# wg-perception/tod

Measured on AMD Instinct MI355X. Metric: frames/sec @ 640x480, 1M-descriptor DB; achieved HBM GB/s on BF-matcher, higher is better.
Workload: dtype fp4 (+-1) x fp4 -> f32 on the matrix cores (exact integers), f32 in the verifier

## Files before the change

include/todhip.h:

```cpp
#ifndef TODHIP_H_
#define TODHIP_H_

#include <stddef.h>
#include <stdint.h>

#ifdef __cplusplus
extern "C" {
#endif

#define TODHIP_VERSION 1

typedef enum {
  TODHIP_OK = 0,
  TODHIP_EINVAL = -1,
  TODHIP_ENODB = -2,
  TODHIP_EHIP = -3,
  TODHIP_ECAPACITY = -4,
  TODHIP_ERANGE = -5,
  TODHIP_ENOMEM = -6,
  TODHIP_ESCRATCH = -7,
  TODHIP_EBUSY = -8,
  TODHIP_ETIMEOUT = -9
} todhip_status;

// ... 3 lines not shown

typedef struct { int32_t queryIdx, trainIdx, imgIdx; float distance; } todhip_dmatch;

typedef struct { uint32_t s[31]; uint32_t f, b; uint64_t draws; } todhip_rng;

typedef struct { uint32_t min_inliers, n_ransac_iterations; float sensor_error; } todhip_verify_params;

typedef struct { uint32_t object; float R[9]; float t[3]; uint32_t inlier_begin, inlier_end; } todhip_pose;

typedef struct {
  uint64_t db_rows, db_objects;
  uint32_t last_nq, last_k, last_matches;
  uint32_t last_objects_verified, last_rounds, last_hypotheses, last_gate_calls, last_poses;
  double   last_match_kernel_ms;
  double   sum_match_kernel_ms;
  uint64_t n_match_kernel_launches;
  uint32_t last_sprint_launches;
  uint32_t last_sprint_rounds;
  uint32_t last_verify_ticks;
  uint32_t last_block_split;
  uint64_t k4x_half_blocks, k4x_half_blocks_completed;
  uint32_t last_fp4_rows;
  uint32_t fp4_rows_builds;
} todhip_counters;

int  todhip_version(void);
int  todhip_create(int device, void* hip_stream, todhip_ctx** out);
void todhip_destroy(todhip_ctx*);
void* todhip_stream(todhip_ctx*);
int  todhip_last_hip_error(const todhip_ctx*);
int  todhip_synchronize(todhip_ctx*);
int  todhip_get_counters(todhip_ctx*, todhip_counters* out);
enum { TODHIP_STREAM_THROUGHPUT = 0, TODHIP_STREAM_LATENCY = 1 };
int  todhip_set_cu_partition(uint32_t latency_cus);
int  todhip_stream_create(int device, int kind, void** stream_out);
int  todhip_stream_destroy(void* stream);
int  todhip_set_kernel_timing(todhip_ctx*, int enable);
enum { TODHIP_ENGINE_AUTO = 0, TODHIP_ENGINE_VALU = 1, TODHIP_ENGINE_MFMA = 2 };
int  todhip_set_matcher_engine(todhip_ctx*, int engine);
int  todhip_set_matcher_block_split(todhip_ctx*, int split);

int todhip_db_load(todhip_ctx*, const todhip_object* objs, uint32_t n_objs, uint32_t desc_bytes,
                   uint32_t shard_rank, uint32_t shard_count, float* spans_out);
int todhip_db_load_device(todhip_ctx*, const todhip_object* objs, uint32_t n_objs, uint32_t desc_bytes,
                          uint32_t shard_rank, uint32_t shard_count, float* spans_out);
int todhip_db_info(const todhip_ctx*, uint64_t* total_rows, uint64_t* shard_first_row, uint64_t* shard_rows,
// ... 251 lines not shown
```

tod_amd/capi.py:

```python
import ctypes as C
import os
import subprocess

import numpy as np

_PKG = os.path.dirname(os.path.abspath(__file__))
LIB_PATH = os.environ.get("TODHIP_LIB_PATH") or os.path.join(_PKG, "libtodhip.so")

OK, EINVAL, ENODB, EHIP, ECAPACITY, ERANGE, ENOMEM, ESCRATCH, EBUSY, ETIMEOUT = 0, -1, -2, -3, -4, -5, -6, -7, -8, -9
FRAME_GRAY8, FRAME_BGR8, FRAME_BGRA8 = 0, 1, 2
PATTERN_ORDER_RANK, PATTERN_ORDER_MATCHER = 0, 1

DMATCH_DTYPE = np.dtype([("queryIdx", "<i4"), ("trainIdx", "<i4"), ("imgIdx", "<i4"), ("distance", "<f4")])


class TodObject(C.Structure):
    _fields_ = [("desc", C.c_void_p), ("pts_xyz", C.c_void_p), ("n", C.c_uint32)]


class Rng(C.Structure):
    _fields_ = [("s", C.c_uint32 * 31), ("f", C.c_uint32), ("b", C.c_uint32), ("draws", C.c_uint64)]


class VerifyParams(C.Structure):
    _fields_ = [("min_inliers", C.c_uint32), ("n_ransac_iterations", C.c_uint32), ("sensor_error", C.c_float)]


class Pose(C.Structure):
    _fields_ = [("object", C.c_uint32), ("R", C.c_float * 9), ("t", C.c_float * 3),
                ("inlier_begin", C.c_uint32), ("inlier_end", C.c_uint32)]


class RoundTrace(C.Structure):
    _fields_ = [("object", C.c_uint32), ("iterations", C.c_uint32), ("best_iteration", C.c_uint32),
                ("best_count", C.c_int32), ("draws_before", C.c_uint64), ("draws_after", C.c_uint64),
                ("n_inlier_kp", C.c_uint32), ("accepted", C.c_uint32)]


class Counters(C.Structure):
    _fields_ = [("db_rows", C.c_uint64), ("db_objects", C.c_uint64), ("last_nq", C.c_uint32), ("last_k", C.c_uint32),
                ("last_matches", C.c_uint32), ("last_objects_verified", C.c_uint32), ("last_rounds", C.c_uint32),
                ("last_hypotheses", C.c_uint32), ("last_gate_calls", C.c_uint32), ("last_poses", C.c_uint32),
                ("last_match_kernel_ms", C.c_double), ("sum_match_kernel_ms", C.c_double),
                ("n_match_kernel_launches", C.c_uint64), ("last_sprint_launches", C.c_uint32), ("last_sprint_rounds", C.c_uint32),
                ("last_verify_ticks", C.c_uint32), ("last_block_split", C.c_uint32), ("k4x_half_blocks", C.c_uint64),
                ("k4x_half_blocks_completed", C.c_uint64), ("last_fp4_rows", C.c_uint32), ("fp4_rows_builds", C.c_uint32)]


class PipelineParams(C.Structure):
    _fields_ = [("struct_size", C.c_uint32), ("frames_per_step", C.c_uint32), ("H", C.c_uint32), ("W", C.c_uint32),
                ("frame_format", C.c_int), ("depth_is_u16", C.c_int), ("K9", C.c_float * 9), ("n_features", C.c_uint32),
                ("n_levels", C.c_uint32), ("scale_factor", C.c_float), ("k", C.c_uint32), ("radius", C.c_uint32),
                ("verify", VerifyParams), ("rng_seed", C.c_uint32), ("orb_workers", C.c_uint32), ("verify_workers", C.c_uint32),
                ("ring_depth", C.c_uint32), ("max_poses_per_frame", C.c_uint32)]


class PipelineStats(C.Structure):
    _fields_ = [("steps", C.c_uint64), ("frames", C.c_uint64), ("keypoints", C.c_uint64), ("poses", C.c_uint64),
                ("orb_s", C.c_double), ("match_issue_s", C.c_double), ("verify_s", C.c_double),
                ("sum_match_kernel_ms", C.c_double), ("n_match_kernel_launches", C.c_uint64)]


class PatternStats(C.Structure):
    _fields_ = [("n_keypoints", C.c_uint32), ("n_candidates", C.c_uint32), ("accepted_in_round", C.c_uint32 * 6)]


EXPORTS = [
    "todhip_version", "todhip_create", "todhip_destroy", "todhip_stream", "todhip_last_hip_error",
    "todhip_synchronize", "todhip_get_counters", "todhip_set_cu_partition", "todhip_stream_create", "todhip_stream_destroy", "todhip_set_kernel_timing", "todhip_set_matcher_engine", "todhip_set_matcher_block_split", "todhip_set_ratio_test", "todhip_db_load", "todhip_db_load_device", "todhip_db_info",
# ... 961 lines not shown
```

tod_amd/csrc/capi.hip:

```cpp
#include <algorithm>
#include <atomic>
#include <cfloat>
#include <cmath>
#include <cstring>
#include <cstdlib>
#include <new>
#include <vector>

#include "ctx.h"

extern "C" {

int todhip_version(void) { return TODHIP_VERSION; }

int todhip_create(int device, void* hip_stream, todhip_ctx** out) {
  if (!out) return TODHIP_EINVAL;
  *out = nullptr;
  todhip_ctx* ctx = new (std::nothrow) todhip_ctx();
  if (!ctx) return TODHIP_ENOMEM;
  ctx->device = device;
  hipError_t e = hipSetDevice(device);
  if (e == hipSuccess) {
    hipDeviceProp_t prop;
    if (hipGetDeviceProperties(&prop, device) == hipSuccess && prop.multiProcessorCount > 0)
// ... 287 lines not shown
  return tod_match_shard_keys(ctx, d_q_desc, nq, k, radius, reinterpret_cast<uint64_t*>(d_keys));
}

int todhip_merge_shards_device_on(todhip_ctx* ctx, void* hip_stream, const void* d_keys_all, uint32_t n_shards, uint32_t nq,
                                  uint32_t k, uint32_t radius, void* d_counts, void* d_matches, void* d_matches_xyz) {
  if (!ctx || !hip_stream) return TODHIP_EINVAL;
  return merge_shards(ctx, reinterpret_cast<hipStream_t>(hip_stream), d_keys_all, n_shards, nq, k, radius, d_counts, d_matches, d_matches_xyz);
}

int todhip_merge_shards_device(todhip_ctx* ctx, const void* d_keys_all, uint32_t n_shards, uint32_t nq, uint32_t k,
                               uint32_t radius, void* d_counts, void* d_matches, void* d_matches_xyz) {
  return merge_shards(ctx, nullptr, d_keys_all, n_shards, nq, k, radius, d_counts, d_matches, d_matches_xyz);
}

int todhip_match_device(todhip_ctx* ctx, const void* d_q_desc, uint32_t nq, uint32_t k, uint32_t radius,
                        void* d_counts, void* d_matches, void* d_matches_xyz) {
  if (!ctx || !d_q_desc || !d_counts || !d_matches || !d_matches_xyz) return TODHIP_EINVAL;
  if (k == 0 || k > 8 || radius == 0) return TODHIP_EINVAL;
  if (ctx->total_rows == 0) return TODHIP_ENODB;
  if (ctx->shard_rows != ctx->total_rows) return TODHIP_EINVAL;
  if (wide_db_with_lsh(ctx)) return TODHIP_EINVAL;
  if (nq == 0) return TODHIP_OK;
  const uint32_t k_in = (ctx->ratio > 0.f && k < 2) ? 2u : k;
  TOD_HIP(ctx->m_keys.reserve(tod_match_lists_bytes(nq, k_in)));
  uint32_t n_lists = 0;
  int rc = tod_match_lists(ctx, d_q_desc, nq, k_in, radius, ctx->m_keys.as<uint64_t>(), &n_lists);
  if (rc != TODHIP_OK) return rc;
  rc = tod_match_finalize(ctx, ctx->m_keys.as<uint64_t>(), n_lists, nq, k_in, k, radius,
                          reinterpret_cast<uint32_t*>(d_counts), reinterpret_cast<todhip_dmatch*>(d_matches),
                          reinterpret_cast<float*>(d_matches_xyz));
  if (rc == TODHIP_OK && ctx->cross_check_q)
    rc = tod_cross_check(ctx, d_q_desc, nq, ctx->cross_check_q, nullptr, k, reinterpret_cast<uint32_t*>(d_counts),
                         reinterpret_cast<todhip_dmatch*>(d_matches), reinterpret_cast<float*>(d_matches_xyz));
  if (rc == TODHIP_OK) { ctx->counters.last_nq = nq; ctx->counters.last_k = k; }
  return rc;
}

int todhip_match(todhip_ctx* ctx, const uint8_t* q_desc, uint32_t nq, uint32_t k, uint32_t radius,
                 uint32_t* row_ptr, todhip_dmatch* matches, float* matches_xyz) {
  if (!ctx || !row_ptr || (nq && (!q_desc || !matches || !matches_xyz))) return TODHIP_EINVAL;
  if (k == 0 || k > 8 || radius == 0) return TODHIP_EINVAL;
  if (ctx->total_rows == 0) return TODHIP_ENODB;
  if (wide_db_with_lsh(ctx)) return TODHIP_EINVAL;
  if (nq == 0) { row_ptr[0] = 0; return TODHIP_OK; }
  TOD_HIP(hipSetDevice(ctx->device));
  const size_t nm = (size_t)nq * k;
  TOD_HIP(ctx->m_q.reserve((size_t)nq * ctx->desc_bytes));
  TOD_HIP(ctx->m_counts.reserve((size_t)nq * sizeof(uint32_t)));
  TOD_HIP(ctx->m_matches.reserve(nm * sizeof(todhip_dmatch)));
  TOD_HIP(ctx->m_xyz.reserve(nm * 3 * sizeof(float)));
  const size_t stage_bytes = (size_t)nq * sizeof(uint32_t) + nm * sizeof(todhip_dmatch) + nm * 3 * sizeof(float);
  TOD_HIP(ctx->h_stage.reserve(stage_bytes));
  TOD_HIP(hipMemcpyAsync(ctx->m_q.p, q_desc, (size_t)nq * ctx->desc_bytes, hipMemcpyHostToDevice, ctx->stream));
// ... 35 lines not shown
```

tod_amd/csrc/ctx.h:

```cpp
#pragma once

#include <hip/hip_runtime.h>

#include <cstdint>
#include <cstdlib>
#include <cstring>
#include <memory>
#include <type_traits>
#include <vector>

#include "../../include/todhip.h"
#include "db_select.h"
#include "fp4_rows.h"
#include "match_split.h"
#include "match_tiles.h"

#define TOD_HIP(call)                                  \
  do {                                                 \
    hipError_t e_ = (call);                            \
    if (e_ != hipSuccess) {                            \
      ctx->last_hip_error = (int)e_;                   \
      return TODHIP_EHIP;                              \
    }                                                  \
  } while (0)

#ifndef TOD_LATENCY_PRIO_LEVEL
#define TOD_LATENCY_PRIO_LEVEL 3
#endif
#define TOD_LATENCY_PRIO() __builtin_amdgcn_s_setprio(TOD_LATENCY_PRIO_LEVEL)

constexpr size_t kDbSlackBytes = 2048;
static_assert(31 * 64 <= kDbSlackBytes, "a 32-row step of the widest binary row must end inside the slack");

struct DevBuf {
  void* p = nullptr;
  size_t cap = 0;
// ... 48 lines not shown
  template <typename T> T* as() const { return reinterpret_cast<T*>(p); }
};

struct TodWs { virtual ~TodWs() {} };
enum TodWsSlot { kWsVerify, kWsOrb, kWsL2, kWsPnp, kWsLsh, kWsLearn, kWsCompact, kWsRadius, kWsCrossCheck, kWsSlots };

struct todhip_ctx {
  int device = 0;
  hipStream_t stream = nullptr;
  bool own_stream = false;
  int last_hip_error = 0;
  int n_cu = 256;

  uint32_t desc_bytes = 0;
  uint64_t total_rows = 0, shard_first = 0, shard_rows = 0;
  uint32_t n_objs = 0;
  DevBuf db_desc;
  DevBuf db_pts;
  DevBuf db_obj_off;
  std::vector<uint32_t> h_obj_off;
  std::vector<float> h_spans;

  DevBuf m_q, m_part, m_keys, m_counts, m_matches, m_xyz, m_bound;
  HostBuf h_stage;
  bool time_kernels = false;
  static constexpr int kEvPairs = 64;
  hipEvent_t evp[2 * kEvPairs] = {};
  uint64_t ev_head = 0, ev_tail = 0;
  todhip_counters counters = {};
  int matcher_engine = TODHIP_ENGINE_AUTO;
  HostBuf k4x_stats_host; DevBuf k4x_stats_dev;
  K4xSplit k4x;
  float ratio = 0.f;
  uint32_t cross_check_q = 0;
  int bit_order_mode = TODHIP_BIT_ORDER_NONE;
  bool bit_order_on = false;
  uint8_t bit_src_of[256];
  DevBuf bit_tab, m_qord;
  bool sel_on = false;
  TodViewTables sel;
  DevBuf view_desc, view_tab;
  DevBuf db_fp4;
  uint64_t rows_gen = 1, fp4_gen = 0;

  std::vector<todhip_round_trace> traces;

// ... 18 lines not shown
  r.s[r.f] += r.s[r.b];
  const uint32_t out = r.s[r.f] >> 1;
  r.f = r.f == 30u ? 0u : r.f + 1u; r.b = r.b == 30u ? 0u : r.b + 1u;
  ++r.draws;
  return out;
}

uint32_t tod_pack_csr(const uint32_t* counts, const todhip_dmatch* m, const float* xyz, uint32_t nq, uint32_t k, uint32_t* row_ptr,
                      todhip_dmatch* matches, float* matches_xyz);
extern "C" hipError_t tod_stream_create(hipStream_t* out, int device, int kind);
extern "C" uint32_t tod_cu_partition();
int tod_timing_begin(todhip_ctx* ctx, int* slot);
int tod_timing_end(todhip_ctx* ctx, int slot);
int tod_timing_drain(todhip_ctx* ctx, uint64_t keep);
struct KernelTimer {
  todhip_ctx* ctx;
  int slot = -1;
  int begin() { return ctx->time_kernels ? tod_timing_begin(ctx, &slot) : TODHIP_OK; }
  int end() { return slot >= 0 ? tod_timing_end(ctx, slot) : TODHIP_OK; }
};
int tod_match_lists(todhip_ctx* ctx, const void* d_q, uint32_t nq, uint32_t k, uint32_t radius, uint64_t* d_lists,
                    uint32_t* n_lists);
size_t tod_match_lists_bytes(uint32_t nq, uint32_t k);
int tod_wide_lists_active(todhip_ctx* ctx, const void* d_q, uint32_t nq, uint32_t k, uint32_t radius, uint64_t* d_lists,
                          uint32_t* n_lists);
template <typename Fn>
int dispatch_k(uint32_t k, Fn fn) {
  switch (k) {
    case 1: return fn(std::integral_constant<int, 1>{});
    case 2: return fn(std::integral_constant<int, 2>{});
    case 3: return fn(std::integral_constant<int, 3>{});
    case 4: return fn(std::integral_constant<int, 4>{});
    case 5: return fn(std::integral_constant<int, 5>{});
    case 6: return fn(std::integral_constant<int, 6>{});
    case 7: return fn(std::integral_constant<int, 7>{});
    case 8: return fn(std::integral_constant<int, 8>{});
    default: return TODHIP_EINVAL;
  }
}
int tod_match_shard_keys(todhip_ctx* ctx, const void* d_q, uint32_t nq, uint32_t k, uint32_t radius, uint64_t* d_keys);
int tod_match_finalize(todhip_ctx* ctx, const uint64_t* d_keys_all, uint32_t n_shards, uint32_t nq, uint32_t k_in, uint32_t k_out,
                       uint32_t radius, uint32_t* d_counts, todhip_dmatch* d_matches, float* d_xyz,
                       hipStream_t stream = nullptr);
int tod_cross_check(todhip_ctx* ctx, const void* d_q, uint32_t nq, uint32_t frame_queries, const uint32_t* frame_nq, uint32_t stride,
                    uint32_t* d_counts, todhip_dmatch* d_matches, float* d_xyz);
int tod_cluster_frames_nocloud(todhip_ctx* ctx, uint32_t F, const float* d_kp_xy, uint32_t nq, const uint32_t* d_counts,
// ... 17 lines not shown
```

tod_amd/csrc/match.hip:

```cpp
#include <algorithm>
#include <cstdio>
#include <cstdlib>
#include <cstring>

#include "ctx.h"
#include "row_ops.h"

namespace {

#include "match_keys.h"
#include "match_valu.h"
#include "match_fp4.h"
#include "match_mfma.h"
#include "match_pair_pack.h"
#include "match_fp4rows.h"
#include "match_merge.h"
#include "match_plan.h"
#include "match_launch.h"

int k4_engine(const todhip_ctx* ctx, uint32_t nq) {
  if (ctx->matcher_engine == TODHIP_ENGINE_VALU) return 0;
  if (ctx->matcher_engine == TODHIP_ENGINE_MFMA) return 1;
  if (match_env().engine == 'v') return 0;
  if (match_env().engine == 'm') return 1;
  return (uint64_t)nq * tod_db_n_rows(ctx) >= (1ull << 24) ? 1 : 0;
}

}

int tod_timing_drain(todhip_ctx* ctx, uint64_t keep) {
  while (ctx->ev_head - ctx->ev_tail > keep) {
    const int i = (int)(ctx->ev_tail % todhip_ctx::kEvPairs);
    TOD_HIP(hipEventSynchronize(ctx->evp[2 * i + 1]));
    float ms = 0.f;
    TOD_HIP(hipEventElapsedTime(&ms, ctx->evp[2 * i], ctx->evp[2 * i + 1]));
    ctx->counters.last_match_kernel_ms = ms;
    ctx->counters.sum_match_kernel_ms += ms;
    ctx->counters.n_match_kernel_launches += 1;
    ++ctx->ev_tail;
  }
// ... 19 lines not shown
  const uint32_t* q = reinterpret_cast<const uint32_t*>(d_q);
  return dispatch_k(k, [&](auto K) { return launch_topk<decltype(K)::value>(ctx, q, nq, radius, d_lists, n_lists); });
}

int tod_match_lists(todhip_ctx* ctx, const void* d_q, uint32_t nq, uint32_t k, uint32_t radius, uint64_t* d_lists,
                    uint32_t* n_lists) {
  const bool wide = ctx->desc_bytes == 64;
  if ((!wide && ctx->desc_bytes != 32) || k == 0 || k > 8 || nq == 0) return TODHIP_EINVAL;
  if (wide && tod_lsh_enabled(ctx)) return TODHIP_EINVAL;
  if (!wide && ctx->bit_order_on) {
    int rc = tod_bit_order_queries(ctx, d_q, nq, &d_q);
    if (rc != TODHIP_OK) return rc;
  }
  if (tod_db_n_rows(ctx) == 0) {
    TOD_HIP(hipMemsetAsync(d_lists, 0xFF, (size_t)nq * k * sizeof(uint64_t), ctx->stream));
    *n_lists = 1;
    return TODHIP_OK;
  }
  int rc = wide ? tod_wide_lists_active(ctx, d_q, nq, k, radius, d_lists, n_lists) : match_lists_active(ctx, d_q, nq, k, radius, d_lists, n_lists);
  if (rc != TODHIP_OK || !ctx->sel_on) return rc;
  return tod_view_remap(ctx, d_lists, (size_t)*n_lists * nq * k);
}

size_t tod_match_lists_bytes(uint32_t nq, uint32_t k) { return (size_t)kMergeGroups * nq * k * sizeof(uint64_t); }

int tod_match_shard_keys(todhip_ctx* ctx, const void* d_q, uint32_t nq, uint32_t k, uint32_t radius, uint64_t* d_keys) {
  if (nq == 0) return TODHIP_OK;
  if (tod_db_n_rows(ctx) == 0) {
    TOD_HIP(hipMemsetAsync(d_keys, 0xFF, (size_t)nq * k * sizeof(uint64_t), ctx->stream));
    return TODHIP_OK;
  }
  TOD_HIP(ctx->m_keys.reserve(tod_match_lists_bytes(nq, k)));
  uint32_t n_lists = 0;
  int rc = tod_match_lists(ctx, d_q, nq, k, radius, ctx->m_keys.as<uint64_t>(), &n_lists);
  if (rc != TODHIP_OK) return rc;
  hipLaunchKernelGGL(select_keys_kernel, dim3((nq + kBlock - 1) / kBlock), dim3(kBlock), 0, ctx->stream,
                     ctx->m_keys.as<uint64_t>(), n_lists, nq, k, d_keys);
  TOD_HIP(hipGetLastError());
  return TODHIP_OK;
}

int tod_match_finalize(todhip_ctx* ctx, const uint64_t* d_keys_all, uint32_t n_shards, uint32_t nq, uint32_t k_in, uint32_t k_out,
                       uint32_t radius, uint32_t* d_counts, todhip_dmatch* d_matches, float* d_xyz, hipStream_t stream) {
  if (nq == 0) return TODHIP_OK;
  const uint32_t blocks = (nq + kBlock - 1) / kBlock;
  hipLaunchKernelGGL(finalize_kernel, dim3(blocks), dim3(kBlock), 0, stream ? stream : ctx->stream, d_keys_all, n_shards, nq, k_in, k_out,
// ... 16 lines not shown
```

tod_amd/csrc/match_launch.h:

```cpp

int k4_engine(const todhip_ctx* ctx, uint32_t nq);

struct MatchEnv {
  char engine;
  int k4_mode;
  int k4_wpc;
  int k4x_wpc;
  int k4x_share;
  int k4x_qt;
  int k4x_half;
  bool k4x_half_debug;
  int k4x_fp4_rows;
  int k4x_fp4_rows_mb;
  int k4x_pairs;
};
inline const MatchEnv& match_env() {
  static const MatchEnv env = [] {
    auto num = [](const char* name, int unset) { const char* e = getenv(name); return e ? atoi(e) : unset; };
    const char* eng = getenv("TODHIP_K4_ENGINE");
    return MatchEnv{eng ? eng[0] : '\0', num("TODHIP_K4_MODE", -1), num("TODHIP_K4_WAVES_PER_CU", 0), num("TODHIP_K4X_WAVES_PER_CU", 0),
                    num("TODHIP_K4X_SHARE", 16), num("TODHIP_K4X_QT", 0), num("TODHIP_K4X_HALF", -1), getenv("TODHIP_K4X_HALF_DEBUG") != nullptr,
                    num("TODHIP_K4X_FP4_ROWS", 1), num("TODHIP_K4X_FP4_ROWS_MB", 512), num("TODHIP_K4X_PAIRS", 1)};
  }();
  return env;
}

inline int fp4_rows_ready(todhip_ctx* ctx, uint32_t n_rows, const uint4** out) {
  const MatchEnv& env = match_env();
  const size_t bytes = fp4_rows_bytes(n_rows);
  if (env.k4x_fp4_rows == 0 || bytes > ((size_t)std::max(0, env.k4x_fp4_rows_mb) << 20) || bytes >= (1ull << 32)) return TODHIP_OK;
  if (ctx->fp4_gen != ctx->rows_gen) {
    TOD_HIP(ctx->db_fp4.reserve(bytes));
    hipLaunchKernelGGL(expand_rows_fp4_kernel, dim3(fp4_rows_steps(n_rows)), dim3(kBlock), 0, ctx->stream,
                       reinterpret_cast<const uint32_t*>(tod_db_rows(ctx)), fp4_rows_steps(n_rows), ctx->db_fp4.as<uint4>());
    TOD_HIP(hipGetLastError());
    ctx->fp4_gen = ctx->rows_gen;
    ++ctx->counters.fp4_rows_builds;
  }
  *out = ctx->db_fp4.as<uint4>();
  return TODHIP_OK;
}

template <int K, int QT>
int launch_topk_mfma_qt(todhip_ctx* ctx, const uint32_t* d_q, uint32_t nq, uint32_t radius, uint64_t* d_lists, uint32_t* n_lists) {
  constexpr bool PF2 = QT < 8;
  const MatchEnv& env = match_env();
  const uint32_t cut = radius >= 256u ? kNoLimit : radius + 1u;
  const uint32_t n_rows = (uint32_t)tod_db_n_rows(ctx);
  const uint32_t n_qw = (nq + 32u * QT - 1u) / (32u * QT), n_qw64 = (nq + 63u) / 64u;
  const uint32_t nq_pad = n_qw64 * 64u;
  uint32_t wpc = 32;
  if ((uint64_t)n_rows * n_qw < (uint64_t)ctx->n_cu * wpc * 1536u) wpc = 16;
  if ((uint64_t)n_rows * n_qw < (uint64_t)ctx->n_cu * 16u * 4096u) wpc = 8;
  if (env.k4x_wpc > 0) wpc = (uint32_t)env.k4x_wpc;
  Tiling t;
  if (!finish_tiling(n_rows, mfma_tile_rows(n_rows, (uint32_t)ctx->n_cu * wpc / n_qw, 256u, true), n_qw, &t)) return TODHIP_EINVAL;
  uint8_t* const d_stored = prepare_lists<K>(ctx, t.n_tiles, nq_pad, n_qw64);
  if (!d_stored) return TODHIP_EHIP;
  KernelTimer timer{ctx};
  if (int rc = timer.begin()) return rc;
  const uint32_t min_split = QT < 4 ? 4u : (cut <= 64u ? 2u : (cut <= 96u ? 3u : 4u));
  if (ctx->k4x.may_split(min_split, env.k4x_half)) {
    if (!ctx->k4x_stats_host.p) {
      TOD_HIP(ctx->k4x_stats_host.reserve(64));
      std::memset(ctx->k4x_stats_host.p, 0, 64);
      TOD_HIP(ctx->k4x_stats_dev.reserve(64));
      TOD_HIP(hipMemsetAsync(ctx->k4x_stats_dev.p, 0, 64, ctx->stream));
    }
    ctx->k4x.take_report(ctx->k4x_stats_host.as<uint32_t>(), ctx->counters, min_split, env.k4x_half, env.k4x_half_debug);
  }
  const uint32_t split = ctx->k4x.next(min_split, env.k4x_half);
  const bool pairs = env.k4x_pairs != 0 && (QT == 6 || nq <= 1024u);
  const int mode = split == 2 ? (pairs ? 2 : 4) : split == 3 ? 3 : cut <= 128u ? 1 : 0;
  ctx->counters.last_block_split = split;
  uint32_t* const d_stats = split < 4 ? ctx->k4x_stats_dev.as<uint32_t>() : nullptr;
  const uint4* rows_fp4 = nullptr;
  if ((QT == 4 || QT == 6) && t.rows_per_tile % 32u == 0u)
    if (int rc = fp4_rows_ready(ctx, n_rows, &rows_fp4)) return rc;
  ctx->counters.last_fp4_rows = rows_fp4 ? 1u : 0u;
  auto launch = [&](auto kern, auto rows) {
    hipLaunchKernelGGL(kern, dim3(t.blocks_per_xcd * 8u), dim3(kBlock), 0, ctx->stream, rows, d_q, n_rows, nq, nq_pad, t.rows_per_tile,
                       t.n_tiles, n_qw, n_qw64, t.blocks_per_xcd, t.tiles_per_xcd, cut, (uint32_t)std::max(2, env.k4x_share),
                       ctx->m_part.as<uint32_t>(), ctx->m_bound.as<uint32_t>(), d_stored, d_stats ? d_stats + 2u * (split - 2u) : nullptr);
  };
  auto launch_mode = [&](auto M) {
    constexpr int MODE = decltype(M)::value;
    if constexpr (QT == 4 || QT == 6)
      if (rows_fp4) return launch(hamming_topk_fp4rows<K, QT, MODE>, rows_fp4);
    launch(hamming_topk_mfma<K, QT, MODE == 4 ? 2 : MODE, PF2>, reinterpret_cast<const uint32_t*>(tod_db_rows(ctx)));
  };
  switch (mode) {
    case 0: launch_mode(std::integral_constant<int, 0>{}); break;
    case 1: launch_mode(std::integral_constant<int, 1>{}); break;
    case 2: launch_mode(std::integral_constant<int, 2>{}); break;
    case 4: launch_mode(std::integral_constant<int, 4>{}); break;
    default: launch_mode(std::integral_constant<int, 3>{}); break;
  }
  if (int rc = timer.end()) return rc;
  if (d_stats) ++ctx->k4x.seq_sent;
  if (nq <= 64u && !d_stats && t.n_tiles >= 256u) return launch_merge_wave<K>(ctx, nq, nq_pad, t, d_stored, n_qw64, d_lists, n_lists);
  return launch_merge<K>(ctx, nq, nq_pad, t, d_stored, n_qw64, d_stats, d_lists, n_lists);
}

template <int K>
int launch_topk_mfma_q32(todhip_ctx* ctx, const uint32_t* d_q, uint32_t nq, uint32_t radius, uint64_t* d_lists, uint32_t* n_lists) {
  const uint32_t cut = radius >= 256u ? kNoLimit : radius + 1u;
  const uint32_t n_rows = (uint32_t)tod_db_n_rows(ctx), n_qw64 = 1u, nq_pad = 64u;
  Tiling t;
  if (!finish_tiling(n_rows, mfma_tile_rows(n_rows, (uint32_t)ctx->n_cu * 32u, 2048u, false), 1u, &t)) return TODHIP_EINVAL;
  uint8_t* const d_stored = prepare_lists<K>(ctx, t.n_tiles, nq_pad, n_qw64);
  if (!d_stored) return TODHIP_EHIP;
  KernelTimer timer{ctx};
  if (int rc = timer.begin()) return rc;
  auto kern = cut <= 128u ? hamming_topk_mfma_q32<K, true> : hamming_topk_mfma_q32<K, false>;
  ctx->counters.last_fp4_rows = 0;
  hipLaunchKernelGGL(kern, dim3((t.n_tiles + kWavesPerBlock - 1) / kWavesPerBlock), dim3(kBlock), 0, ctx->stream,
                     reinterpret_cast<const uint32_t*>(tod_db_rows(ctx)), d_q, n_rows, nq, nq_pad, t.rows_per_tile, t.n_tiles, n_qw64, cut,
                     (uint32_t)std::max(4, match_env().k4x_share), ctx->m_part.as<uint32_t>(), ctx->m_bound.as<uint32_t>(), d_stored);
  if (int rc = timer.end()) return rc;
  return launch_merge_wave<K>(ctx, nq, nq_pad, t, d_stored, n_qw64, d_lists, n_lists);
}

template <int K>
int launch_topk_mfma(todhip_ctx* ctx, const uint32_t* d_q, uint32_t nq, uint32_t radius, uint64_t* d_lists, uint32_t* n_lists) {
  const int env_qt = match_env().k4x_qt;
  if (nq <= 32u && !(env_qt > 0))
    return launch_topk_mfma_q32<K>(ctx, d_q, nq, radius, d_lists, n_lists);
  constexpr int kMaxQT = K <= 2 ? 8 : (K <= 5 ? 6 : 4);
  auto padded = [&](uint32_t qt) { return (uint64_t)((nq + 32u * qt - 1u) / (32u * qt) * (32u * qt)); };
  int qt = kMaxQT >= 6 ? 6 : 4;
  if (kMaxQT >= 8 && padded(8) * 103u < padded(6) * 100u) qt = 8;
  if (qt > 4 && padded(4) * 103u < padded((uint32_t)qt) * 100u) qt = 4;
  if (padded(2) * 103u < padded((uint32_t)qt) * 100u) qt = 2;
  if (nq <= 2048u && qt > 4) qt = 4;
  if ((env_qt == 2 || env_qt == 4 || env_qt == 6 || env_qt == 8) && env_qt <= kMaxQT) qt = env_qt;
  if (qt == 8) return launch_topk_mfma_qt<K, (kMaxQT >= 8 ? 8 : 4)>(ctx, d_q, nq, radius, d_lists, n_lists);
  if (qt == 6) return launch_topk_mfma_qt<K, (kMaxQT >= 6 ? 6 : 4)>(ctx, d_q, nq, radius, d_lists, n_lists);
  if (qt == 2) return launch_topk_mfma_qt<K, 2>(ctx, d_q, nq, radius, d_lists, n_lists);
  return launch_topk_mfma_qt<K, 4>(ctx, d_q, nq, radius, d_lists, n_lists);
}

template <int K>
int launch_topk(todhip_ctx* ctx, const uint32_t* d_q, uint32_t nq, uint32_t radius, uint64_t* d_lists, uint32_t* n_lists) {
  if (k4_engine(ctx, nq) == 1) return launch_topk_mfma<K>(ctx, d_q, nq, radius, d_lists, n_lists);
  const MatchEnv& env = match_env();
  const uint32_t cut = radius >= 256u ? 0xFFFFFFFFu : radius + 1u;
  const uint32_t n_rows = (uint32_t)tod_db_n_rows(ctx);
  const uint32_t n_qw = (nq + 63u) / 64u;
  const uint32_t nq_pad = n_qw * 64u;
  uint32_t n_tiles;
  if (env.k4_wpc > 0) {
    n_tiles = (uint32_t)ctx->n_cu * (uint32_t)env.k4_wpc / n_qw;
  } else {
    n_tiles = std::max(3u * (uint32_t)ctx->n_cu * (uint32_t)kWavesPerCU / n_qw, (n_rows + 2047u) / 2048u);
    n_tiles = std::min(n_tiles, 8192u);
  }
  if (n_tiles < 1) n_tiles = 1;
  if (n_tiles >= 8) n_tiles = (n_tiles + 7u) & ~7u;
  uint32_t rows_per_tile = (n_rows + n_tiles - 1) / n_tiles;
  rows_per_tile = ((rows_per_tile + 2 * kGroupRows - 1) / (2 * kGroupRows)) * (2 * kGroupRows);
  if (rows_per_tile < 64) rows_per_tile = 64;
  Tiling t;
// ... 16 lines not shown
```

tod_amd/csrc/match_merge.h:

```cpp

template <int K>
__global__ __launch_bounds__(kBlock) void merge_tiles_kernel(const uint32_t* __restrict__ part, uint32_t nq,
                                                             uint32_t nq_pad, uint32_t n_tiles,
                                                             uint32_t rows_per_tile, uint64_t first_global_row,
                                                             uint32_t n_groups, const uint8_t* __restrict__ stored,
                                                             uint32_t n_qw, uint64_t* __restrict__ keys,
                                                             const uint32_t* stat_src = nullptr, uint32_t* stat_dst = nullptr,
                                                             uint32_t stat_seq = 0) {
  TOD_LATENCY_PRIO();
  const uint32_t qi = blockIdx.x * kBlock + threadIdx.x;
  const uint32_t grp = blockIdx.y;
  if (stat_dst && qi == 0u && grp == 0u) {
    for (int i = 0; i < 4; ++i) stat_dst[i] = __hip_atomic_load(stat_src + i, __ATOMIC_RELAXED, __HIP_MEMORY_SCOPE_AGENT);
    __threadfence_system();
    stat_dst[4] = stat_seq;
  }
  if (qi >= nq) return;
  uint64_t best[K];
#pragma unroll
  for (int j = 0; j < K; ++j) best[j] = ~0ull;
#pragma unroll 4
  for (uint32_t t = grp; t < n_tiles; t += n_groups) {
    if (stored[(size_t)t * n_qw + (qi >> 6)] != 0) continue;
    uint32_t pk[K];
// ... 57 lines not shown
    for (int j = 0; j < K; ++j) keys[((size_t)grp * nq + qi) * K + j] = best[j];
  }
}

__global__ __launch_bounds__(kBlock) void select_keys_kernel(const uint64_t* __restrict__ lists, uint32_t n_lists,
                                                             uint32_t nq, uint32_t k, uint64_t* __restrict__ keys) {
  TOD_LATENCY_PRIO();
  const uint32_t qi = blockIdx.x * kBlock + threadIdx.x;
  if (qi >= nq) return;
  uint64_t last = 0;
  bool have_last = false;
  for (uint32_t j = 0; j < k; ++j) {
    const uint64_t nxt = next_key_over_lists(lists, n_lists, nq, qi, k, last, have_last);
    keys[(size_t)qi * k + j] = nxt;
    if (nxt == ~0ull) {
      for (uint32_t jj = j + 1; jj < k; ++jj) keys[(size_t)qi * k + jj] = ~0ull;
      break;
    }
    last = nxt;
    have_last = true;
  }
}

__global__ __launch_bounds__(kBlock) void finalize_kernel(const uint64_t* __restrict__ keys_all, uint32_t n_shards,
                                                          uint32_t nq, uint32_t k_in, uint32_t k_out, uint32_t radius, float ratio,
                                                          const uint32_t* __restrict__ obj_off, uint32_t n_objs,
                                                          const float* __restrict__ pts,
                                                          uint32_t* __restrict__ counts,
                                                          todhip_dmatch* __restrict__ matches,
                                                          float* __restrict__ xyz) {
  TOD_LATENCY_PRIO();
  const uint32_t qi = blockIdx.x * kBlock + threadIdx.x;
  if (qi >= nq) return;
  uint64_t picked[9];
  const uint32_t want = ratio > 0.f ? max(k_out, 2u) : k_out;
  uint32_t n_picked = 0;
  uint64_t last = 0;
  bool have_last = false;
  for (uint32_t j = 0; j < want; ++j) {
    const uint64_t nxt = next_key_over_lists(keys_all, n_shards, nq, qi, k_in, last, have_last);
    if (nxt == ~0ull) break;
    last = nxt;
    have_last = true;
    picked[n_picked++] = nxt;
  }
  if (ratio > 0.f && n_picked >= 2u && !((float)(uint32_t)(picked[0] >> 32) < ratio * (float)(uint32_t)(picked[1] >> 32))) n_picked = 0;
  uint32_t kept = 0;
  for (uint32_t j = 0; j < n_picked && j < k_out; ++j) {
    const uint32_t d = (uint32_t)(picked[j] >> 32);
    if ((float)d > (float)radius) break;
    store_match(qi, d, (uint32_t)picked[j], (size_t)qi * k_out + kept, obj_off, n_objs, pts, matches, xyz);
    ++kept;
  }
  counts[qi] = kept;
}
```

tod_amd/csrc/match_plan.h:

```cpp

inline bool finish_tiling(uint32_t n_rows, uint32_t rows_per_tile, uint32_t n_qw, Tiling* t) {
  if (rows_per_tile > kLocalMask) return false;
  *t = tile_plan(n_rows, rows_per_tile, n_qw, kWavesPerBlock, kMergeGroups);
  return true;
}

template <int K>
uint8_t* prepare_lists(todhip_ctx* ctx, uint32_t n_tiles, uint32_t nq_pad, uint32_t n_qw64) {
  const size_t bound_bytes = (size_t)nq_pad * sizeof(uint32_t), flag_bytes = (size_t)n_tiles * n_qw64;
  hipError_t e = ctx->m_part.reserve((size_t)n_tiles * K * nq_pad * sizeof(uint32_t));
  if (e == hipSuccess) e = ctx->m_bound.reserve(bound_bytes + flag_bytes);
  if (e == hipSuccess) e = hipMemsetAsync(ctx->m_bound.p, 0xFF, bound_bytes + flag_bytes, ctx->stream);
  if (e != hipSuccess) { ctx->last_hip_error = (int)e; return nullptr; }
  return ctx->m_bound.as<uint8_t>() + bound_bytes;
}

template <int K>
int launch_merge(todhip_ctx* ctx, uint32_t nq, uint32_t nq_pad, const Tiling& t, const uint8_t* d_stored, uint32_t n_qw64,
                 const uint32_t* d_stats, uint64_t* d_lists, uint32_t* n_lists) {
  hipLaunchKernelGGL(merge_tiles_kernel<K>, dim3((nq + kBlock - 1) / kBlock, t.groups), dim3(kBlock), 0, ctx->stream,
                     ctx->m_part.as<uint32_t>(), nq, nq_pad, t.n_tiles, t.rows_per_tile, tod_db_first_row(ctx), t.groups, d_stored, n_qw64, d_lists,
                     d_stats, d_stats ? ctx->k4x_stats_host.as<uint32_t>() : (uint32_t*)nullptr, d_stats ? ctx->k4x.seq_sent : 0u);
  TOD_HIP(hipGetLastError());
  *n_lists = t.groups;
  return TODHIP_OK;
}

template <int K>
int launch_merge_wave(todhip_ctx* ctx, uint32_t nq, uint32_t nq_pad, const Tiling& t, const uint8_t* d_stored, uint32_t n_qw64,
                      uint64_t* d_lists, uint32_t* n_lists) {
  hipLaunchKernelGGL(merge_tiles_wave_kernel<K>, dim3((nq + kWavesPerBlock - 1) / kWavesPerBlock, t.groups), dim3(kBlock), 0, ctx->stream,
                     ctx->m_part.as<uint32_t>(), nq, nq_pad, t.n_tiles, t.rows_per_tile, tod_db_first_row(ctx), t.groups, d_stored, n_qw64, d_lists);
  TOD_HIP(hipGetLastError());
  *n_lists = t.groups;
  return TODHIP_OK;
}
// ... 1 lines not shown
```

Before: 25040.

## Fuse tile merge with finalize epilogue and skip per-call bound memset

Adds a direct MFMA match path that merges per-tile top-K partials and writes final DMatch/xyz output in one kernel, instead of writing intermediate 64-bit lists and running a separate finalize kernel. The fused kernel also restores the bound/stored-flag buffer to 0xFF on exit, so the next call can skip the hipMemsetAsync when the buffer is already clean. This removes one kernel launch, a global round trip of the list buffer, and a memset per frame. The cost is extra coupling: correctness now depends on the previous fused kernel having fully reset the scratch flags.

```diff
diff --git a/include/todhip.h b/include/todhip.h
--- a/include/todhip.h
+++ b/include/todhip.h
@@ -49,6 +49,8 @@
   uint64_t k4x_half_blocks, k4x_half_blocks_completed;
   uint32_t last_fp4_rows;
   uint32_t fp4_rows_builds;
+  uint32_t last_match_epilogue;
+  uint32_t bound_memsets;
 } todhip_counters;
 
 int  todhip_version(void);
diff --git a/tod_amd/capi.py b/tod_amd/capi.py
--- a/tod_amd/capi.py
+++ b/tod_amd/capi.py
@@ -44,7 +44,8 @@
                 ("last_match_kernel_ms", C.c_double), ("sum_match_kernel_ms", C.c_double),
                 ("n_match_kernel_launches", C.c_uint64), ("last_sprint_launches", C.c_uint32), ("last_sprint_rounds", C.c_uint32),
                 ("last_verify_ticks", C.c_uint32), ("last_block_split", C.c_uint32), ("k4x_half_blocks", C.c_uint64),
-                ("k4x_half_blocks_completed", C.c_uint64), ("last_fp4_rows", C.c_uint32), ("fp4_rows_builds", C.c_uint32)]
+                ("k4x_half_blocks_completed", C.c_uint64), ("last_fp4_rows", C.c_uint32), ("fp4_rows_builds", C.c_uint32),
+                ("last_match_epilogue", C.c_uint32), ("bound_memsets", C.c_uint32)]
 
 
 class PipelineParams(C.Structure):
diff --git a/tod_amd/csrc/capi.hip b/tod_amd/csrc/capi.hip
--- a/tod_amd/csrc/capi.hip
+++ b/tod_amd/csrc/capi.hip
@@ -333,13 +333,19 @@
   if (wide_db_with_lsh(ctx)) return TODHIP_EINVAL;
   if (nq == 0) return TODHIP_OK;
   const uint32_t k_in = (ctx->ratio > 0.f && k < 2) ? 2u : k;
-  TOD_HIP(ctx->m_keys.reserve(tod_match_lists_bytes(nq, k_in)));
-  uint32_t n_lists = 0;
-  int rc = tod_match_lists(ctx, d_q_desc, nq, k_in, radius, ctx->m_keys.as<uint64_t>(), &n_lists);
+  bool done = false;
+  int rc = tod_match_direct(ctx, d_q_desc, nq, k_in, k, radius, reinterpret_cast<uint32_t*>(d_counts),
+                            reinterpret_cast<todhip_dmatch*>(d_matches), reinterpret_cast<float*>(d_matches_xyz), &done);
   if (rc != TODHIP_OK) return rc;
-  rc = tod_match_finalize(ctx, ctx->m_keys.as<uint64_t>(), n_lists, nq, k_in, k, radius,
-                          reinterpret_cast<uint32_t*>(d_counts), reinterpret_cast<todhip_dmatch*>(d_matches),
-                          reinterpret_cast<float*>(d_matches_xyz));
+  if (!done) {
+    TOD_HIP(ctx->m_keys.reserve(tod_match_lists_bytes(nq, k_in)));
+    uint32_t n_lists = 0;
+    rc = tod_match_lists(ctx, d_q_desc, nq, k_in, radius, ctx->m_keys.as<uint64_t>(), &n_lists);
+    if (rc != TODHIP_OK) return rc;
+    rc = tod_match_finalize(ctx, ctx->m_keys.as<uint64_t>(), n_lists, nq, k_in, k, radius,
+                            reinterpret_cast<uint32_t*>(d_counts), reinterpret_cast<todhip_dmatch*>(d_matches),
+                            reinterpret_cast<float*>(d_matches_xyz));
+  }
   if (rc == TODHIP_OK && ctx->cross_check_q)
     rc = tod_cross_check(ctx, d_q_desc, nq, ctx->cross_check_q, nullptr, k, reinterpret_cast<uint32_t*>(d_counts),
                          reinterpret_cast<todhip_dmatch*>(d_matches), reinterpret_cast<float*>(d_matches_xyz));
diff --git a/tod_amd/csrc/ctx.h b/tod_amd/csrc/ctx.h
--- a/tod_amd/csrc/ctx.h
+++ b/tod_amd/csrc/ctx.h
@@ -12,6 +12,7 @@
 #include "../../include/todhip.h"
 #include "db_select.h"
 #include "fp4_rows.h"
+#include "match_bound_extent.h"
 #include "match_split.h"
 #include "match_tiles.h"
 
@@ -106,6 +107,7 @@
   std::vector<float> h_spans;
 
   DevBuf m_q, m_part, m_keys, m_counts, m_matches, m_xyz, m_bound;
+  BoundExtent m_bound_clean;
   HostBuf h_stage;
   bool time_kernels = false;
   static constexpr int kEvPairs = 64;
@@ -170,6 +172,8 @@
 int tod_match_lists(todhip_ctx* ctx, const void* d_q, uint32_t nq, uint32_t k, uint32_t radius, uint64_t* d_lists,
                     uint32_t* n_lists);
 size_t tod_match_lists_bytes(uint32_t nq, uint32_t k);
+int tod_match_direct(todhip_ctx* ctx, const void* d_q, uint32_t nq, uint32_t k_in, uint32_t k_out, uint32_t radius, uint32_t* d_counts,
+                     todhip_dmatch* d_matches, float* d_xyz, bool* done);
 int tod_wide_lists_active(todhip_ctx* ctx, const void* d_q, uint32_t nq, uint32_t k, uint32_t radius, uint64_t* d_lists,
                           uint32_t* n_lists);
 template <typename Fn>
diff --git a/tod_amd/csrc/match.hip b/tod_amd/csrc/match.hip
--- a/tod_amd/csrc/match.hip
+++ b/tod_amd/csrc/match.hip
@@ -16,6 +16,7 @@
 #include "match_fp4rows.h"
 #include "match_merge.h"
 #include "match_plan.h"
+#include "match_epilogue.h"
 #include "match_launch.h"
 
 int k4_engine(const todhip_ctx* ctx, uint32_t nq) {
@@ -81,6 +82,30 @@
   return tod_view_remap(ctx, d_lists, (size_t)*n_lists * nq * k);
 }
 
+int tod_match_direct(todhip_ctx* ctx, const void* d_q, uint32_t nq, uint32_t k_in, uint32_t k_out, uint32_t radius, uint32_t* d_counts,
+                     todhip_dmatch* d_matches, float* d_xyz, bool* done) {
+  *done = false;
+  ctx->counters.last_match_epilogue = 0;
+  if (match_env().epilogue == 0 || ctx->desc_bytes != 32 || k_in == 0 || k_in > 8 || nq == 0) return TODHIP_OK;
+  if (tod_lsh_enabled(ctx) || ctx->sel_on || tod_db_n_rows(ctx) == 0) return TODHIP_OK;
+  if (k4_engine(ctx, nq) != 1 || !mfma_takes_qt(nq)) return TODHIP_OK;
+  if (ctx->bit_order_on) {
+    int rc = tod_bit_order_queries(ctx, d_q, nq, &d_q);
+    if (rc != TODHIP_OK) return rc;
+  }
+  MatchOut out{k_out, radius, d_counts, d_matches, d_xyz, false};
+  const uint32_t search_radius = ctx->ratio > 0.f ? 256u : radius;
+  const uint32_t* q = reinterpret_cast<const uint32_t*>(d_q);
+  uint32_t n_lists = 0;
+  int rc = dispatch_k(k_in, [&](auto K) { return launch_topk_mfma<decltype(K)::value>(ctx, q, nq, search_radius, nullptr, &n_lists, &out); });
+  if (rc != TODHIP_OK) return rc;
+  if (!out.taken)
+    rc = tod_match_finalize(ctx, ctx->m_keys.as<uint64_t>(), n_lists, nq, k_in, k_out, radius, d_counts, d_matches, d_xyz);
+  ctx->counters.last_match_epilogue = out.taken ? 1u : 0u;
+  *done = true;
+  return rc;
+}
+
 size_t tod_match_lists_bytes(uint32_t nq, uint32_t k) { return (size_t)kMergeGroups * nq * k * sizeof(uint64_t); }
 
 int tod_match_shard_keys(todhip_ctx* ctx, const void* d_q, uint32_t nq, uint32_t k, uint32_t radius, uint64_t* d_keys) {
diff --git a/tod_amd/csrc/match_bound_extent.h b/tod_amd/csrc/match_bound_extent.h
--- /dev/null
+++ b/tod_amd/csrc/match_bound_extent.h
@@ -0,0 +1,19 @@
+#pragma once
+#include <algorithm>
+#include <cstddef>
+
+struct BoundExtent {
+  size_t clean = 0;
+  size_t held = 0;
+
+  void reallocated() { clean = held = 0; }
+
+  bool begin(size_t need, bool restoring) {
+    const bool fill = !restoring || need > clean;
+    held = restoring ? std::max(clean, need) : 0;
+    clean = 0;
+    return fill;
+  }
+
+  void restored() { clean = held; held = 0; }
+};
diff --git a/tod_amd/csrc/match_epilogue.h b/tod_amd/csrc/match_epilogue.h
--- /dev/null
+++ b/tod_amd/csrc/match_epilogue.h
@@ -0,0 +1,93 @@
+
+constexpr int kEpiGroups = 4;
+
+struct MatchOut {
+  uint32_t k_out, radius;
+  uint32_t* counts;
+  todhip_dmatch* matches;
+  float* xyz;
+  bool taken;
+};
+
+template <int K>
+__global__ __launch_bounds__(kBlock) void merge_finalize_kernel(const uint32_t* __restrict__ part, uint32_t nq, uint32_t nq_pad, uint32_t n_tiles,
+                                                                uint32_t rows_per_tile, uint64_t first_global_row, uint8_t* stored,
+                                                                uint32_t n_qw64, uint32_t* bound, uint32_t k_out, uint32_t radius, float ratio,
+                                                                const uint32_t* __restrict__ obj_off, uint32_t n_objs,
+                                                                const float* __restrict__ pts, uint32_t* __restrict__ counts,
+                                                                todhip_dmatch* __restrict__ matches, float* __restrict__ xyz,
+                                                                const uint32_t* stat_src, uint32_t* stat_dst, uint32_t stat_seq) {
+  TOD_LATENCY_PRIO();
+  static_assert(kBlock == 64 * kEpiGroups, "a workgroup is 64 queries x kEpiGroups tile groups");
+  __shared__ uint64_t lists[kEpiGroups * K * 64];
+  const uint32_t q = threadIdx.x & 63u, grp = threadIdx.x >> 6, qw = blockIdx.x;
+  const uint32_t qi = qw * 64u + q;
+  if (stat_dst && threadIdx.x == 0u && qw == 0u) {
+    for (int i = 0; i < 4; ++i) stat_dst[i] = __hip_atomic_load(stat_src + i, __ATOMIC_RELAXED, __HIP_MEMORY_SCOPE_AGENT);
+    __threadfence_system();
+    stat_dst[4] = stat_seq;
+  }
+  uint64_t best[K];
+#pragma unroll
+  for (int j = 0; j < K; ++j) best[j] = ~0ull;
+  if (qi < nq) {
+#pragma unroll 4
+    for (uint32_t t = grp; t < n_tiles; t += kEpiGroups) {
+      if (stored[(size_t)t * n_qw64 + qw] != 0) continue;
+      uint32_t pk[K];
+#pragma unroll
+      for (int j = 0; j < K; ++j) pk[j] = part[((size_t)t * K + j) * nq_pad + qi];
+#pragma unroll
+      for (int j = 0; j < K; ++j) {
+        uint64_t key = pk[j] == 0xFFFFFFFFu
+                           ? ~0ull
+                           : (((uint64_t)(pk[j] >> kLocalBits) << 32) |
+                              (first_global_row + (uint64_t)t * rows_per_tile + (pk[j] & kLocalMask)));
+#pragma unroll
+        for (int s2 = 0; s2 < K; ++s2) {
+          uint64_t lo = key < best[s2] ? key : best[s2];
+          key = key < best[s2] ? best[s2] : key;
+          best[s2] = lo;
+        }
+      }
+    }
+  }
+#pragma unroll
+  for (int j = 0; j < K; ++j) lists[(grp * K + j) * 64u + q] = best[j];
+  __syncthreads();
+  if (grp == 0u && qi < nq) {
+    uint64_t picked[9];
+    const uint32_t want = ratio > 0.f ? max(k_out, 2u) : k_out;
+    uint32_t n_picked = 0, heads = 0;
+    for (uint32_t j = 0; j < want; ++j) {
+      uint64_t nxt = ~0ull;
+      uint32_t from = 0;
+#pragma unroll
+      for (uint32_t g = 0; g < (uint32_t)kEpiGroups; ++g) {
+        const uint32_t h = (heads >> (8u * g)) & 0xFFu;
+        if (h >= (uint32_t)K) continue;
+        const uint64_t v = lists[(g * K + h) * 64u + q];
+        if (v < nxt) { nxt = v; from = g; }
+      }
+      if (nxt == ~0ull) break;
+      heads += 1u << (8u * from);
+      picked[n_picked++] = nxt;
+    }
+    finalize_tail(qi, picked, n_picked, k_out, radius, ratio, obj_off, n_objs, pts, counts, matches, xyz);
+  }
+  for (uint32_t t = threadIdx.x; t < n_tiles; t += kBlock) stored[(size_t)t * n_qw64 + qw] = 0xFFu;
+  if (threadIdx.x < 64u) bound[qi] = 0xFFFFFFFFu;
+}
+
+template <int K>
+int launch_merge_finalize(todhip_ctx* ctx, uint32_t nq, uint32_t nq_pad, const Tiling& t, uint8_t* d_stored, uint32_t n_qw64,
+                          const uint32_t* d_stats, MatchOut* out) {
+  hipLaunchKernelGGL(merge_finalize_kernel<K>, dim3(n_qw64), dim3(kBlock), 0, ctx->stream, ctx->m_part.as<uint32_t>(), nq, nq_pad, t.n_tiles,
+                     t.rows_per_tile, tod_db_first_row(ctx), d_stored, n_qw64, ctx->m_bound.as<uint32_t>(), out->k_out, out->radius, ctx->ratio,
+                     ctx->db_obj_off.as<uint32_t>(), ctx->n_objs, ctx->db_pts.as<float>(), out->counts, out->matches, out->xyz, d_stats,
+                     d_stats ? ctx->k4x_stats_host.as<uint32_t>() : (uint32_t*)nullptr, d_stats ? ctx->k4x.seq_sent : 0u);
+  TOD_HIP(hipGetLastError());
+  ctx->m_bound_clean.restored();
+  out->taken = true;
+  return TODHIP_OK;
+}
diff --git a/tod_amd/csrc/match_launch.h b/tod_amd/csrc/match_launch.h
--- a/tod_amd/csrc/match_launch.h
+++ b/tod_amd/csrc/match_launch.h
@@ -13,6 +13,7 @@
   int k4x_fp4_rows;
   int k4x_fp4_rows_mb;
   int k4x_pairs;
+  int epilogue;
 };
 inline const MatchEnv& match_env() {
   static const MatchEnv env = [] {
@@ -20,7 +21,7 @@
     const char* eng = getenv("TODHIP_K4_ENGINE");
     return MatchEnv{eng ? eng[0] : '\0', num("TODHIP_K4_MODE", -1), num("TODHIP_K4_WAVES_PER_CU", 0), num("TODHIP_K4X_WAVES_PER_CU", 0),
                     num("TODHIP_K4X_SHARE", 16), num("TODHIP_K4X_QT", 0), num("TODHIP_K4X_HALF", -1), getenv("TODHIP_K4X_HALF_DEBUG") != nullptr,
-                    num("TODHIP_K4X_FP4_ROWS", 1), num("TODHIP_K4X_FP4_ROWS_MB", 512), num("TODHIP_K4X_PAIRS", 1)};
+                    num("TODHIP_K4X_FP4_ROWS", 1), num("TODHIP_K4X_FP4_ROWS_MB", 512), num("TODHIP_K4X_PAIRS", 1), num("TODHIP_MATCH_EPILOGUE", 1)};
   }();
   return env;
 }
@@ -42,7 +43,8 @@
 }
 
 template <int K, int QT>
-int launch_topk_mfma_qt(todhip_ctx* ctx, const uint32_t* d_q, uint32_t nq, uint32_t radius, uint64_t* d_lists, uint32_t* n_lists) {
+int launch_topk_mfma_qt(todhip_ctx* ctx, const uint32_t* d_q, uint32_t nq, uint32_t radius, uint64_t* d_lists, uint32_t* n_lists,
+                        MatchOut* direct = nullptr) {
   constexpr bool PF2 = QT < 8;
   const MatchEnv& env = match_env();
   const uint32_t cut = radius >= 256u ? kNoLimit : radius + 1u;
@@ -55,10 +57,6 @@
   if (env.k4x_wpc > 0) wpc = (uint32_t)env.k4x_wpc;
   Tiling t;
   if (!finish_tiling(n_rows, mfma_tile_rows(n_rows, (uint32_t)ctx->n_cu * wpc / n_qw, 256u, true), n_qw, &t)) return TODHIP_EINVAL;
-  uint8_t* const d_stored = prepare_lists<K>(ctx, t.n_tiles, nq_pad, n_qw64);
-  if (!d_stored) return TODHIP_EHIP;
-  KernelTimer timer{ctx};
-  if (int rc = timer.begin()) return rc;
   const uint32_t min_split = QT < 4 ? 4u : (cut <= 64u ? 2u : (cut <= 96u ? 3u : 4u));
   if (ctx->k4x.may_split(min_split, env.k4x_half)) {
     if (!ctx->k4x_stats_host.p) {
@@ -70,10 +68,16 @@
     ctx->k4x.take_report(ctx->k4x_stats_host.as<uint32_t>(), ctx->counters, min_split, env.k4x_half, env.k4x_half_debug);
   }
   const uint32_t split = ctx->k4x.next(min_split, env.k4x_half);
+  uint32_t* const d_stats = split < 4 ? ctx->k4x_stats_dev.as<uint32_t>() : nullptr;
+  const bool wave_merge = nq <= 64u && !d_stats && t.n_tiles >= 256u;
+  const bool fused = direct && !wave_merge;
+  uint8_t* const d_stored = prepare_lists<K>(ctx, t.n_tiles, nq_pad, n_qw64, fused);
+  if (!d_stored) return TODHIP_EHIP;
+  KernelTimer timer{ctx};
+  if (int rc = timer.begin()) return rc;
   const bool pairs = env.k4x_pairs != 0 && (QT == 6 || nq <= 1024u);
   const int mode = split == 2 ? (pairs ? 2 : 4) : split == 3 ? 3 : cut <= 128u ? 1 : 0;
   ctx->counters.last_block_split = split;
-  uint32_t* const d_stats = split < 4 ? ctx->k4x_stats_dev.as<uint32_t>() : nullptr;
   const uint4* rows_fp4 = nullptr;
   if ((QT == 4 || QT == 6) && t.rows_per_tile % 32u == 0u)
     if (int rc = fp4_rows_ready(ctx, n_rows, &rows_fp4)) return rc;
@@ -98,7 +102,12 @@
   }
   if (int rc = timer.end()) return rc;
   if (d_stats) ++ctx->k4x.seq_sent;
-  if (nq <= 64u && !d_stats && t.n_tiles >= 256u) return launch_merge_wave<K>(ctx, nq, nq_pad, t, d_stored, n_qw64, d_lists, n_lists);
+  if (fused) return launch_merge_finalize<K>(ctx, nq, nq_pad, t, d_stored, n_qw64, d_stats, direct);
+  if (direct) {
+    TOD_HIP(ctx->m_keys.reserve(tod_match_lists_bytes(nq, K)));
+    d_lists = ctx->m_keys.as<uint64_t>();
+  }
+  if (wave_merge) return launch_merge_wave<K>(ctx, nq, nq_pad, t, d_stored, n_qw64, d_lists, n_lists);
   return launch_merge<K>(ctx, nq, nq_pad, t, d_stored, n_qw64, d_stats, d_lists, n_lists);
 }
 
@@ -121,10 +130,13 @@
   return launch_merge_wave<K>(ctx, nq, nq_pad, t, d_stored, n_qw64, d_lists, n_lists);
 }
 
+inline bool mfma_takes_qt(uint32_t nq) { return nq > 32u || match_env().k4x_qt > 0; }
+
 template <int K>
-int launch_topk_mfma(todhip_ctx* ctx, const uint32_t* d_q, uint32_t nq, uint32_t radius, uint64_t* d_lists, uint32_t* n_lists) {
+int launch_topk_mfma(todhip_ctx* ctx, const uint32_t* d_q, uint32_t nq, uint32_t radius, uint64_t* d_lists, uint32_t* n_lists,
+                     MatchOut* direct = nullptr) {
   const int env_qt = match_env().k4x_qt;
-  if (nq <= 32u && !(env_qt > 0))
+  if (!mfma_takes_qt(nq))
     return launch_topk_mfma_q32<K>(ctx, d_q, nq, radius, d_lists, n_lists);
   constexpr int kMaxQT = K <= 2 ? 8 : (K <= 5 ? 6 : 4);
   auto padded = [&](uint32_t qt) { return (uint64_t)((nq + 32u * qt - 1u) / (32u * qt) * (32u * qt)); };
@@ -134,10 +146,10 @@
   if (padded(2) * 103u < padded((uint32_t)qt) * 100u) qt = 2;
   if (nq <= 2048u && qt > 4) qt = 4;
   if ((env_qt == 2 || env_qt == 4 || env_qt == 6 || env_qt == 8) && env_qt <= kMaxQT) qt = env_qt;
-  if (qt == 8) return launch_topk_mfma_qt<K, (kMaxQT >= 8 ? 8 : 4)>(ctx, d_q, nq, radius, d_lists, n_lists);
-  if (qt == 6) return launch_topk_mfma_qt<K, (kMaxQT >= 6 ? 6 : 4)>(ctx, d_q, nq, radius, d_lists, n_lists);
-  if (qt == 2) return launch_topk_mfma_qt<K, 2>(ctx, d_q, nq, radius, d_lists, n_lists);
-  return launch_topk_mfma_qt<K, 4>(ctx, d_q, nq, radius, d_lists, n_lists);
+  if (qt == 8) return launch_topk_mfma_qt<K, (kMaxQT >= 8 ? 8 : 4)>(ctx, d_q, nq, radius, d_lists, n_lists, direct);
+  if (qt == 6) return launch_topk_mfma_qt<K, (kMaxQT >= 6 ? 6 : 4)>(ctx, d_q, nq, radius, d_lists, n_lists, direct);
+  if (qt == 2) return launch_topk_mfma_qt<K, 2>(ctx, d_q, nq, radius, d_lists, n_lists, direct);
+  return launch_topk_mfma_qt<K, 4>(ctx, d_q, nq, radius, d_lists, n_lists, direct);
 }
 
 template <int K>
diff --git a/tod_amd/csrc/match_merge.h b/tod_amd/csrc/match_merge.h
--- a/tod_amd/csrc/match_merge.h
+++ b/tod_amd/csrc/match_merge.h
@@ -103,6 +103,21 @@
   }
 }
 
+__device__ __forceinline__ void finalize_tail(uint32_t qi, const uint64_t (&picked)[9], uint32_t n_picked, uint32_t k_out, uint32_t radius,
+                                              float ratio, const uint32_t* __restrict__ obj_off, uint32_t n_objs,
+                                              const float* __restrict__ pts, uint32_t* __restrict__ counts,
+                                              todhip_dmatch* __restrict__ matches, float* __restrict__ xyz) {
+  if (ratio > 0.f && n_picked >= 2u && !((float)(uint32_t)(picked[0] >> 32) < ratio * (float)(uint32_t)(picked[1] >> 32))) n_picked = 0;
+  uint32_t kept = 0;
+  for (uint32_t j = 0; j < n_picked && j < k_out; ++j) {
+    const uint32_t d = (uint32_t)(picked[j] >> 32);
+    if ((float)d > (float)radius) break;
+    store_match(qi, d, (uint32_t)picked[j], (size_t)qi * k_out + kept, obj_off, n_objs, pts, matches, xyz);
+    ++kept;
+  }
+  counts[qi] = kept;
+}
+
 __global__ __launch_bounds__(kBlock) void finalize_kernel(const uint64_t* __restrict__ keys_all, uint32_t n_shards,
                                                           uint32_t nq, uint32_t k_in, uint32_t k_out, uint32_t radius, float ratio,
                                                           const uint32_t* __restrict__ obj_off, uint32_t n_objs,
@@ -125,13 +140,5 @@
     have_last = true;
     picked[n_picked++] = nxt;
   }
-  if (ratio > 0.f && n_picked >= 2u && !((float)(uint32_t)(picked[0] >> 32) < ratio * (float)(uint32_t)(picked[1] >> 32))) n_picked = 0;
-  uint32_t kept = 0;
-  for (uint32_t j = 0; j < n_picked && j < k_out; ++j) {
-    const uint32_t d = (uint32_t)(picked[j] >> 32);
-    if ((float)d > (float)radius) break;
-    store_match(qi, d, (uint32_t)picked[j], (size_t)qi * k_out + kept, obj_off, n_objs, pts, matches, xyz);
-    ++kept;
-  }
-  counts[qi] = kept;
+  finalize_tail(qi, picked, n_picked, k_out, radius, ratio, obj_off, n_objs, pts, counts, matches, xyz);
 }
diff --git a/tod_amd/csrc/match_plan.h b/tod_amd/csrc/match_plan.h
--- a/tod_amd/csrc/match_plan.h
+++ b/tod_amd/csrc/match_plan.h
@@ -6,12 +6,17 @@
 }
 
 template <int K>
-uint8_t* prepare_lists(todhip_ctx* ctx, uint32_t n_tiles, uint32_t nq_pad, uint32_t n_qw64) {
+uint8_t* prepare_lists(todhip_ctx* ctx, uint32_t n_tiles, uint32_t nq_pad, uint32_t n_qw64, bool restoring = false) {
   const size_t bound_bytes = (size_t)nq_pad * sizeof(uint32_t), flag_bytes = (size_t)n_tiles * n_qw64;
   hipError_t e = ctx->m_part.reserve((size_t)n_tiles * K * nq_pad * sizeof(uint32_t));
+  const size_t cap_before = ctx->m_bound.cap;
   if (e == hipSuccess) e = ctx->m_bound.reserve(bound_bytes + flag_bytes);
-  if (e == hipSuccess) e = hipMemsetAsync(ctx->m_bound.p, 0xFF, bound_bytes + flag_bytes, ctx->stream);
-  if (e != hipSuccess) { ctx->last_hip_error = (int)e; return nullptr; }
+  if (ctx->m_bound.cap != cap_before) ctx->m_bound_clean.reallocated();
+  if (e == hipSuccess && ctx->m_bound_clean.begin(bound_bytes + flag_bytes, restoring)) {
+    e = hipMemsetAsync(ctx->m_bound.p, 0xFF, bound_bytes + flag_bytes, ctx->stream);
+    ++ctx->counters.bound_memsets;
+  }
+  if (e != hipSuccess) { ctx->m_bound_clean.reallocated(); ctx->last_hip_error = (int)e; return nullptr; }
   return ctx->m_bound.as<uint8_t>() + bound_bytes;
 }
 
```

After: 25350, median of 6. 1.01x the previous value.
